# ModelCloud/GPTQModel

Hardware: NVIDIA H100
Metric: W4A16 g128 QuantLinear: decode tok/s + prefill TFLOPS vs HBM/TC roofline (higher is better)
Workload: dtype f16

## Files before the change

gptqmodel_b200/csrc/b2q_dequant.cuh:

```cuda
#pragma once
#include "b2q_common.cuh"

namespace b2q {

struct SZRaw {
  uint32_t s;
  uint32_t zw;
};

template <typename T, int BITS, bool ASYM>
__device__ __forceinline__ SZRaw load_sz(const T* __restrict__ scales, const uint32_t* __restrict__ qzeros, int g,
                                         int n, int N) {
  SZRaw r;
  r.s = *reinterpret_cast<const uint16_t*>(scales + (size_t)g * N + n);
  r.zw = 0;
  if (ASYM) {
    constexpr int PF = 32 / BITS;
    r.zw = qzeros[(size_t)g * (N / PF) + n / PF];
  }
  return r;
}

template <typename T, int BITS>
struct Dequant;

template <>
struct Dequant<__half, 4> {
  __device__ static __forceinline__ void run(const uint4& pv, uint32_t slo16, int zlo_i, uint32_t shi16, int zhi_i,
                                             uint4 (&lo)[2], uint4 (&hi)[2]) {
    const uint32_t slu = slo16 | (slo16 << 16), shu = shi16 | (shi16 << 16);
    const __half2 sl = *reinterpret_cast<const __half2*>(&slu), sh = *reinterpret_cast<const __half2*>(&shu);
    const __half2 zlo = __float2half2_rn(1024.f + (float)zlo_i);
    const __half2 zhi = __float2half2_rn(-(64.f + (float)zhi_i));
    const __half2 sixteenth = __float2half2_rn(0.0625f);
    const uint32_t w[4] = {pv.x, pv.y, pv.z, pv.w};
    uint32_t l[8], u[8];
#pragma unroll
    for (int s4 = 0; s4 < 4; ++s4) {
      uint32_t h[4];
      ET<__half>::unpack_w4(w[s4], h);
      __half2 v0 = __hmul2(__hsub2(*reinterpret_cast<__half2*>(&h[0]), zlo), sl);
      __half2 v1 = __hmul2(__hfma2(*reinterpret_cast<__half2*>(&h[1]), sixteenth, zhi), sh);
      __half2 v2 = __hmul2(__hsub2(*reinterpret_cast<__half2*>(&h[2]), zlo), sl);
      __half2 v3 = __hmul2(__hfma2(*reinterpret_cast<__half2*>(&h[3]), sixteenth, zhi), sh);
      l[2 * s4] = *reinterpret_cast<uint32_t*>(&v0);
      l[2 * s4 + 1] = *reinterpret_cast<uint32_t*>(&v2);
      u[2 * s4] = *reinterpret_cast<uint32_t*>(&v1);
      u[2 * s4 + 1] = *reinterpret_cast<uint32_t*>(&v3);
    }
    lo[0] = make_uint4(l[0], l[1], l[2], l[3]);
    lo[1] = make_uint4(l[4], l[5], l[6], l[7]);
    hi[0] = make_uint4(u[0], u[1], u[2], u[3]);
    hi[1] = make_uint4(u[4], u[5], u[6], u[7]);
  }
};

template <>
struct Dequant<__nv_bfloat16, 4> {
  __device__ static __forceinline__ void run(const uint4& pv, uint32_t slo16, int zlo_i, uint32_t shi16, int zhi_i,
                                             uint4 (&lo)[2], uint4 (&hi)[2]) {
    const uint32_t slu = slo16 | (slo16 << 16), shu = shi16 | (shi16 << 16);
    const __nv_bfloat162 sl = *reinterpret_cast<const __nv_bfloat162*>(&slu);
    const __nv_bfloat162 sh = *reinterpret_cast<const __nv_bfloat162*>(&shu);
    const __nv_bfloat162 zl = __float2bfloat162_rn(128.f + (float)zlo_i);
    const __nv_bfloat162 zh = __float2bfloat162_rn(128.f + (float)zhi_i);
    const uint32_t w[4] = {pv.x, pv.y, pv.z, pv.w};
    uint32_t l[8], u[8];
#pragma unroll
    for (int s4 = 0; s4 < 4; ++s4) {
      uint32_t h[4];
      ET<__nv_bfloat16>::unpack_w4(w[s4], h);
      __nv_bfloat162 v0 = __hmul2(__hsub2(*reinterpret_cast<__nv_bfloat162*>(&h[0]), zl), sl);
      __nv_bfloat162 v1 = __hmul2(__hsub2(*reinterpret_cast<__nv_bfloat162*>(&h[1]), zh), sh);
      __nv_bfloat162 v2 = __hmul2(__hsub2(*reinterpret_cast<__nv_bfloat162*>(&h[2]), zl), sl);
      __nv_bfloat162 v3 = __hmul2(__hsub2(*reinterpret_cast<__nv_bfloat162*>(&h[3]), zh), sh);
      l[2 * s4] = *reinterpret_cast<uint32_t*>(&v0);
      l[2 * s4 + 1] = *reinterpret_cast<uint32_t*>(&v2);
      u[2 * s4] = *reinterpret_cast<uint32_t*>(&v1);
      u[2 * s4 + 1] = *reinterpret_cast<uint32_t*>(&v3);
    }
    lo[0] = make_uint4(l[0], l[1], l[2], l[3]);
    lo[1] = make_uint4(l[4], l[5], l[6], l[7]);
    hi[0] = make_uint4(u[0], u[1], u[2], u[3]);
    hi[1] = make_uint4(u[4], u[5], u[6], u[7]);
  }
};

template <>
struct Dequant<__half, 8> {
  __device__ static __forceinline__ void run(const uint4& pv, uint32_t s16, int z, uint4 (&o)[2]) {
    const uint32_t s2u = s16 | (s16 << 16);
    const __half2 s2 = *reinterpret_cast<const __half2*>(&s2u);
    const __half2 zb = __float2half2_rn(1024.f + (float)z);
    const uint32_t w[4] = {pv.x, pv.y, pv.z, pv.w};
    uint32_t r[8];
#pragma unroll
    for (int t = 0; t < 4; ++t) {
      uint32_t p0 = __byte_perm(w[t], 0x64006400u, 0x7150);
      uint32_t p1 = __byte_perm(w[t], 0x64006400u, 0x7352);
      __half2 v0 = __hmul2(__hsub2(*reinterpret_cast<__half2*>(&p0), zb), s2);
      __half2 v1 = __hmul2(__hsub2(*reinterpret_cast<__half2*>(&p1), zb), s2);
      r[2 * t] = *reinterpret_cast<uint32_t*>(&v0);
      r[2 * t + 1] = *reinterpret_cast<uint32_t*>(&v1);
    }
    o[0] = make_uint4(r[0], r[1], r[2], r[3]);
    o[1] = make_uint4(r[4], r[5], r[6], r[7]);
  }
};

template <>
struct Dequant<__nv_bfloat16, 8> {
  __device__ static __forceinline__ void run(const uint4& pv, uint32_t s16, int z, uint4 (&o)[2]) {
    const float s = __uint_as_float(s16 << 16);
    const uint32_t w[4] = {pv.x, pv.y, pv.z, pv.w};
    uint32_t r[8];
#pragma unroll
    for (int t = 0; t < 4; ++t) {
      const float q0 = (float)((int)(w[t] & 0xFFu) - z), q1 = (float)((int)((w[t] >> 8) & 0xFFu) - z);
      const float q2 = (float)((int)((w[t] >> 16) & 0xFFu) - z), q3 = (float)((int)(w[t] >> 24) - z);
      r[2 * t] = ET<__nv_bfloat16>::pack2(q0 * s, q1 * s);
      r[2 * t + 1] = ET<__nv_bfloat16>::pack2(q2 * s, q3 * s);
    }
    o[0] = make_uint4(r[0], r[1], r[2], r[3]);
    o[1] = make_uint4(r[4], r[5], r[6], r[7]);
  }
};


}
```

gptqmodel_b200/csrc/b2q_gemm.cu:

```cuda
#include <cuda.h>

#include "b2q_common.cuh"
#include "b2q_dequant.cuh"
#include "b2q_gemm.cuh"
#include "b2q_internal.h"
#include "b2q_wgmma.cuh"

namespace b2q {

template <typename T, int BITS, bool ASYM, int STAGES>
__global__ void __launch_bounds__(G_THREADS, 1)
    gemm_kernel(const __grid_constant__ CUtensorMap tmap_x, const __grid_constant__ GemmSets S, int M, int K,
                int gshc) {
  using C = GemmCfg<BITS, STAGES>;
  using E = ET<T>;
  extern __shared__ uint8_t smem_raw[];
  const uint32_t smem_base = (smem_u32(smem_raw) + 1023u) & ~1023u;
  uint8_t* smem = smem_raw + (smem_base - smem_u32(smem_raw));

  const uint32_t sA = smem_base;
  const uint32_t sB = sA + STAGES * C::A_BYTES;
  const uint32_t sP = sB + STAGES * C::B_BYTES;
  const uint32_t sBar = sP + STAGES * C::P_BYTES;
  const uint32_t bar_full = sBar, bar_bready = sBar + 8 * STAGES, bar_empty = sBar + 16 * STAGES;

  int set = 0, tn = blockIdx.x;
  if (S.nsets > 1 && tn >= S.tn_end[0]) {
    set = (S.nsets > 2 && tn >= S.tn_end[1]) ? 2 : 1;
    tn -= S.tn_end[set - 1];
  }
  const int N = S.N[set];
  const uint4* __restrict__ packed = S.packed[set];
  const T* __restrict__ scales = reinterpret_cast<const T*>(S.scales[set]);
  const uint32_t* __restrict__ qzeros = S.qzeros[set];

  const int warp = threadIdx.x >> 5, lane = threadIdx.x & 31;
  const int NT = N >> 5;
  const int n0 = tn * G_BN, m0 = blockIdx.y * G_BM;
  const int nt0 = n0 >> 5;
  const int ntiles = min(4, NT - nt0);
  const int nkb = K / G_BK;

  if (threadIdx.x == 0) {
    prefetch_tmap(&tmap_x);
    for (int s = 0; s < STAGES; ++s) {
      mbar_init(bar_full + 8 * s, 1);
      mbar_init(bar_bready + 8 * s, G_DQ_THREADS);
      mbar_init(bar_empty + 8 * s, 1);
    }
    fence_mbar_init();
  }
  __syncthreads();

  if (warp == 8) {
    if (lane == 0) {
      const int FT = N >> 4, ft0 = n0 >> 4;
      const uint32_t pbytes4 = (uint32_t)min(8, FT - ft0) * 512u;
      const uint32_t pbytes8 = (uint32_t)ntiles * C::SUB * 512u;
      for (int kb = 0; kb < nkb; ++kb) {
        const int s = kb % STAGES;
        const uint32_t ph = (kb / STAGES) & 1;
        mbar_wait(bar_empty + 8 * s, ph ^ 1);
        const int g0 = (2 * kb) >> gshc, g1 = (2 * kb + 1) >> gshc;
        const int nrows = (g1 != g0) ? 2 : 1;
        const uint32_t sbytes = (uint32_t)min(G_BN, N - n0) * 2u, zbytes = ASYM ? sbytes / 4u : 0u;
        mbar_expect_tx(bar_full + 8 * s,
                       C::A_BYTES + (BITS == 4 ? pbytes4 + nrows * (sbytes + zbytes) : 2 * pbytes8));
        tma_load_2d(sA + s * C::A_BYTES, &tmap_x, bar_full + 8 * s, kb * G_BK, m0);
        if (BITS == 4) {
          bulk_load(sP + s * C::P_BYTES, packed + ((size_t)kb * FT + ft0) * 32, pbytes4, bar_full + 8 * s);
          for (int r = 0; r < nrows; ++r) {
            const int gr = r ? g1 : g0;
            bulk_load(sP + s * C::P_BYTES + 4096 + r * 320, scales + (size_t)gr * N + n0, sbytes, bar_full + 8 * s);
            if (ASYM)
              bulk_load(sP + s * C::P_BYTES + 4096 + r * 320 + 256, qzeros + (size_t)gr * (N >> 3) + (n0 >> 3),
                        zbytes, bar_full + 8 * s);
          }
        } else {
#pragma unroll
          for (int j = 0; j < 2; ++j)
            bulk_load(sP + s * C::P_BYTES + j * C::P_CHUNK_BYTES,
                      packed + ((size_t)(kb * 2 + j) * NT + nt0) * C::SUB * 32, pbytes8, bar_full + 8 * s);
        }
      }
    }
  } else if (warp < 4) {
    float acc[2][G_BN / 2];
#pragma unroll
    for (int mb = 0; mb < 2; ++mb)
#pragma unroll
      for (int i = 0; i < G_BN / 2; ++i) acc[mb][i] = 0.f;
    for (int kb = 0; kb < nkb; ++kb) {
      const int s = kb % STAGES;
      const uint32_t ph = (kb / STAGES) & 1;
      mbar_wait(bar_full + 8 * s, ph);
      mbar_wait(bar_bready + 8 * s, ph);
      wgmma_fence();
      const uint64_t bdesc = wgmma_desc_k_sw128(sB + s * C::B_BYTES);
      const uint64_t adesc = wgmma_desc_k_sw128(sA + s * C::A_BYTES);
#pragma unroll
      for (int k = 0; k < G_BK / 16; ++k) {
#pragma unroll
        for (int mb = 0; mb < 2; ++mb)
          Wgmma<E::FMT, G_BN>::mma(acc[mb], adesc + 512 * mb + 2 * k, bdesc + 2 * k, (kb | k) != 0 ? 1u : 0u);
      }
      wgmma_commit();
      wgmma_wait<1>();
      if (kb > 0 && threadIdx.x == 0) mbar_arrive(bar_empty + 8 * ((kb - 1) % STAGES));
    }
    wgmma_wait<0>();
#pragma unroll
    for (int mb = 0; mb < 2; ++mb) wgmma_fence_regs(acc[mb]);

    const T* __restrict__ bias = reinterpret_cast<const T*>(S.bias[set]);
    T* __restrict__ out = reinterpret_cast<T*>(S.out[set]);
#pragma unroll
    for (int mb = 0; mb < 2; ++mb) {
#pragma unroll
      for (int h = 0; h < 2; ++h) {
        const int row = m0 + 64 * mb + 16 * warp + (lane >> 2) + 8 * h;
        if (row >= M) continue;
        T* dst = out + (size_t)row * N;
#pragma unroll
        for (int j = 0; j < G_BN / 8; ++j) {
          const int col = n0 + 8 * j + 2 * (lane & 3);
          if (col >= N) continue;
          float f0 = acc[mb][4 * j + 2 * h], f1 = acc[mb][4 * j + 2 * h + 1];
          if (bias != nullptr) {
            f0 = E::to_f(E::from_f(f0)) + E::to_f(bias[col]);
            f1 = E::to_f(E::from_f(f1)) + E::to_f(bias[col + 1]);
          }
          *reinterpret_cast<uint32_t*>(dst + col) = E::pack2(f0, f1);
        }
      }
    }
  } else {
    const int t = threadIdx.x - G_MMA_THREADS;
    constexpr int PF = 32 / BITS;
    constexpr int ZSYM = 1 << (BITS - 1);
    if (BITS == 4) {
      const int lp = t & 31, g = lp >> 2, tt = lp & 3;
      int f[4];
      f[0] = (t >> 5) * 16 + g;
      f[1] = f[0] + 8;
      f[2] = f[0] + 64;
      f[3] = f[0] + 72;
      for (int kb = 0; kb < nkb; ++kb) {
        const int s = kb % STAGES;
        const uint32_t ph = (kb / STAGES) & 1;
        mbar_wait(bar_full + 8 * s, ph);
        const uint8_t* pst = smem + (sP - smem_base) + s * C::P_BYTES;
        const uint4* pj = reinterpret_cast<const uint4*>(pst);
        const int grow = ((2 * kb + (tt >> 1)) >> gshc) - ((2 * kb) >> gshc);
        const uint8_t* srow = pst + 4096 + grow * 320;
#pragma unroll
        for (int u = 0; u < 2; ++u) {
          const uint4 pv = pj[t + u * 128];
          const uint32_t s_lo = *reinterpret_cast<const uint16_t*>(srow + f[2 * u] * 2);
          const uint32_t s_hi = *reinterpret_cast<const uint16_t*>(srow + f[2 * u + 1] * 2);
          int zl = ZSYM, zh = ZSYM;
          if (ASYM) {
            const uint32_t zwl = *reinterpret_cast<const uint32_t*>(srow + 256 + (f[2 * u] >> 3) * 4);
            const uint32_t zwh = *reinterpret_cast<const uint32_t*>(srow + 256 + (f[2 * u + 1] >> 3) * 4);
            zl = (int)((zwl >> (4 * g)) & 15u);
            zh = (int)((zwh >> (4 * g)) & 15u);
          }
          uint4 lo[2], hi[2];
          Dequant<T, 4>::run(pv, s_lo, zl, s_hi, zh, lo, hi);
          const uint32_t sw = (uint32_t)g;
          const uint32_t rlo = sB + s * C::B_BYTES + f[2 * u] * 128;
          const uint32_t rhi = rlo + 8 * 128;
#pragma unroll
          for (int c = 0; c < 2; ++c) {
            const uint32_t off = (((uint32_t)(2 * tt + c)) ^ sw) << 4;
            asm volatile("st.shared.v4.u32 [%0], {%1,%2,%3,%4};" ::"r"(rlo + off), "r"(lo[c].x), "r"(lo[c].y),
                         "r"(lo[c].z), "r"(lo[c].w)
                         : "memory");
            asm volatile("st.shared.v4.u32 [%0], {%1,%2,%3,%4};" ::"r"(rhi + off), "r"(hi[c].x), "r"(hi[c].y),
                         "r"(hi[c].z), "r"(hi[c].w)
                         : "memory");
          }
        }
        fence_proxy_async_smem();
        mbar_arrive(bar_bready + 8 * s);
      }
    } else {
      const int n = n0 + t;
      const int nsafe = (n < N) ? n : 0;
      const int ntl = t >> 5;
      SZRaw cur[2], nxt[2];
      cur[0] = load_sz<T, BITS, ASYM>(scales, qzeros, 0, nsafe, N);
      cur[1] = load_sz<T, BITS, ASYM>(scales, qzeros, 1 >> gshc, nsafe, N);
      for (int kb = 0; kb < nkb; ++kb) {
        const int s = kb % STAGES;
        const uint32_t ph = (kb / STAGES) & 1;
        if (kb + 1 < nkb) {
          nxt[0] = load_sz<T, BITS, ASYM>(scales, qzeros, (2 * kb + 2) >> gshc, nsafe, N);
          nxt[1] = load_sz<T, BITS, ASYM>(scales, qzeros, (2 * kb + 3) >> gshc, nsafe, N);
        }
        mbar_wait(bar_full + 8 * s, ph);
        const uint32_t brow = sB + s * C::B_BYTES + t * 128;
        const uint32_t sw = (uint32_t)(t & 7);
#pragma unroll
        for (int j = 0; j < 2; ++j) {
          int z = ZSYM;
          if (ASYM) z = (int)((cur[j].zw >> (BITS * (nsafe % PF))) & ((1u << BITS) - 1));
          const uint4* pj = reinterpret_cast<const uint4*>(smem + (sP - smem_base) + s * C::P_BYTES +
                                                           j * C::P_CHUNK_BYTES);
#pragma unroll
          for (int h = 0; h < 2; ++h) {
            const uint4 pv = pj[(ntl * 2 + h) * 32 + lane];
            uint4 o[2];
            Dequant<T, 8>::run(pv, cur[j].s, z, o);
#pragma unroll
            for (int c = 0; c < 2; ++c) {
              const uint32_t addr = brow + (((uint32_t)(j * 4 + h * 2 + c) ^ sw) << 4);
              asm volatile("st.shared.v4.u32 [%0], {%1,%2,%3,%4};" ::"r"(addr), "r"(o[c].x), "r"(o[c].y),
                           "r"(o[c].z), "r"(o[c].w)
                           : "memory");
            }
          }
        }
        fence_proxy_async_smem();
        mbar_arrive(bar_bready + 8 * s);
        cur[0] = nxt[0];
        cur[1] = nxt[1];
      }
    }
  }
}

typedef CUresult (*EncodeTiledFn)(CUtensorMap*, CUtensorMapDataType, cuuint32_t, void*, const cuuint64_t*,
                                  const cuuint64_t*, const cuuint32_t*, const cuuint32_t*, CUtensorMapInterleave,
                                  CUtensorMapSwizzle, CUtensorMapL2promotion, CUtensorMapFloatOOBfill);

static EncodeTiledFn get_encode_fn() {
  static EncodeTiledFn fn = nullptr;
  if (fn == nullptr) {
    void* p = nullptr;
    cudaDriverEntryPointQueryResult qres;
    if (cudaGetDriverEntryPoint("cuTensorMapEncodeTiled", &p, cudaEnableDefault, &qres) == cudaSuccess &&
        qres == cudaDriverEntryPointSuccess)
      fn = reinterpret_cast<EncodeTiledFn>(p);
  }
  return fn;
}

int make_x_tmap_box(CUtensorMap* map, const void* x, int M, int K, int dtype, int box_rows) {
  struct Entry {
    const void* x;
    int M, K, dtype, box;
    CUtensorMap map;
  };
  constexpr int NCACHE = 16;
  static thread_local Entry cache[NCACHE];
  static thread_local int next = 0, filled = 0;
  for (int i = 0; i < filled; ++i) {
    const Entry& c = cache[i];
    if (c.x == x && c.M == M && c.K == K && c.dtype == dtype && c.box == box_rows) {
      *map = c.map;
      return 0;
    }
  }
  EncodeTiledFn enc = get_encode_fn();
  if (enc == nullptr) {
    set_error("b2q_gemm: cuTensorMapEncodeTiled not available from the driver");
    return -1;
  }
  cuuint64_t gdim[2] = {(cuuint64_t)K, (cuuint64_t)M};
  cuuint64_t gstride[1] = {(cuuint64_t)K * 2};
  cuuint32_t box[2] = {(cuuint32_t)G_BK, (cuuint32_t)box_rows};
  cuuint32_t estr[2] = {1, 1};
  CUresult r = enc(map, dtype == 0 ? CU_TENSOR_MAP_DATA_TYPE_FLOAT16 : CU_TENSOR_MAP_DATA_TYPE_BFLOAT16, 2,
                   const_cast<void*>(x), gdim, gstride, box, estr, CU_TENSOR_MAP_INTERLEAVE_NONE,
                   CU_TENSOR_MAP_SWIZZLE_128B, CU_TENSOR_MAP_L2_PROMOTION_L2_256B,
                   CU_TENSOR_MAP_FLOAT_OOB_FILL_NONE);
  if (r != CUDA_SUCCESS) {
    set_error("b2q_gemm: cuTensorMapEncodeTiled failed (%d) for x=%p M=%d K=%d box=%d", (int)r, x, M, K, box_rows);
    return -1;
  }
  Entry& e = cache[next];
  e.x = x;
  e.M = M;
  e.K = K;
  e.dtype = dtype;
  e.box = box_rows;
  e.map = *map;
  next = (next + 1) % NCACHE;
  if (filled < NCACHE) ++filled;
  return 0;
}

int make_x_tmap(CUtensorMap* map, const void* x, int M, int K, int dtype) {
  return make_x_tmap_box(map, x, M, K, dtype, 128);
}

int gemm_gshc(const MmArgs& a) {
  if (a.group_size == 32) return 0;
  if (a.group_size == 64) return 1;
  if (a.group_size == 128) return 2;
  return 31;
}


template <typename T, int BITS, bool ASYM, int STAGES>
static int launch_gemm_t(const MmArgs& a, const void* x, const GemmSets& S) {
  using C = GemmCfg<BITS, STAGES>;
  CUtensorMap tmap;
  if (make_x_tmap(&tmap, x, a.M, a.K, a.dtype) != 0) return -1;
  auto kern = gemm_kernel<T, BITS, ASYM, STAGES>;
  static int smem_opted[32] = {};
  if (int e = ensure_dyn_smem(kern, C::SMEM_BYTES, smem_opted, "b2q_gemm")) return e;
  dim3 grid(S.tn_end[S.nsets - 1], (a.M + G_BM - 1) / G_BM, 1);
  kern<<<grid, G_THREADS, C::SMEM_BYTES, a.stream>>>(tmap, S, a.M, a.K, gemm_gshc(a));
  return (int)cudaGetLastError();
}

static int launch_gemm_sets(const MmArgs& a, const void* x, const GemmSets& S) {
  const bool asym = S.qzeros[0] != nullptr;
#define B2Q_GEMM_CASE(T, BITS, ST) \
  (asym ? launch_gemm_t<T, BITS, true, ST>(a, x, S) : launch_gemm_t<T, BITS, false, ST>(a, x, S))
  if (a.dtype == 0) return a.bits == 4 ? B2Q_GEMM_CASE(__half, 4, 4) : B2Q_GEMM_CASE(__half, 8, 4);
  return a.bits == 4 ? B2Q_GEMM_CASE(__nv_bfloat16, 4, 4) : B2Q_GEMM_CASE(__nv_bfloat16, 8, 4);
#undef B2Q_GEMM_CASE
}

int launch_gemm_multi(const MmArgs& a, const void* x, int nsets, const void* const* packed, const void* const* scales,
                      const int32_t* const* qzeros, const void* const* bias, void* const* out, const int* Ns) {
  if (nsets < 1 || nsets > G_MAX_SETS) {
    set_error("b2q_gemm_multi: nsets=%d out of range (1..%d)", nsets, G_MAX_SETS);
    return -1;
  }
  if (a.K % G_BK != 0) {
    set_error("b2q_gemm_multi: K=%d must be a multiple of %d", a.K, G_BK);
    return -1;
  }
  GemmSets S = {};
  S.nsets = nsets;
  int tn = 0;
  for (int i = 0; i < nsets; ++i) {
    if (Ns[i] <= 0 || Ns[i] % 32 != 0 || packed[i] == nullptr || scales[i] == nullptr || out[i] == nullptr ||
        ((qzeros[i] != nullptr) != (qzeros[0] != nullptr))) {
      set_error("b2q_gemm_multi: set %d unsupported (N=%d; all sets share K, group size and symmetry)", i, Ns[i]);
      return -1;
    }
    tn += (Ns[i] + G_BN - 1) / G_BN;
    S.tn_end[i] = tn;
    S.N[i] = Ns[i];
    S.packed[i] = (const uint4*)packed[i];
    S.scales[i] = scales[i];
    S.qzeros[i] = (const uint32_t*)qzeros[i];
    S.bias[i] = bias[i];
    S.out[i] = out[i];
  }
  for (int i = nsets; i < G_MAX_SETS; ++i) S.tn_end[i] = tn;
  return launch_gemm_sets(a, x, S);
}

int launch_gemm(const MmArgs& a) {
  if (a.K % G_BK != 0) {
    set_error("b2q_gemm: K=%d must be a multiple of %d", a.K, G_BK);
    return -1;
  }
  const void* x = a.x;
  if (a.perm != nullptr) {
    const size_t need = (size_t)a.M * a.K * 2;
    if (a.workspace == nullptr || a.workspace_bytes < need) {
      set_error("b2q_gemm: act-order needs a %zu-byte workspace (got %zu)", need, a.workspace_bytes);
      return -1;
    }
    int e = launch_permute_cols(a.x, a.perm, a.workspace, a.M, a.K, a.stream);
    if (e != 0) return e;
    x = a.workspace;
  }
  if (a.M <= 128 && env().midm && midm_supported(a)) return launch_midm(a, x);
  const void* packed = a.packed;
  const void* scales = a.scales;
  const int32_t* qzeros = (const int32_t*)a.qzeros;
  const void* bias = a.bias;
  void* out = a.out;
  return launch_gemm_multi(a, x, 1, &packed, &scales, &qzeros, &bias, &out, &a.N);
}

}
```

gptqmodel_b200/csrc/b2q_gemm.cuh:

```cuda
#pragma once
#include "b2q_common.cuh"

namespace b2q {

constexpr int G_BM = 128;
constexpr int G_BN = 128;
constexpr int G_BK = 64;
constexpr int G_MMA_THREADS = 128;
constexpr int G_DQ_THREADS = 128;
constexpr int G_THREADS = G_MMA_THREADS + G_DQ_THREADS + 32;

template <int BITS, int STAGES>
struct GemmCfg {
  static constexpr int SUB = BITS / 4;
  static constexpr int A_BYTES = G_BM * G_BK * 2;
  static constexpr int B_BYTES = G_BN * G_BK * 2;
  static constexpr int P_CHUNK_BYTES = 4 * SUB * 512;
  static constexpr int P_BYTES = 2 * P_CHUNK_BYTES + (BITS == 4 ? 1024 : 0);
  static constexpr int STAGE_BYTES = A_BYTES + B_BYTES + P_BYTES;
  static constexpr int BAR_BYTES = 256;
  static constexpr int SMEM_BYTES = STAGES * STAGE_BYTES + BAR_BYTES + 1024;
  static_assert(SMEM_BYTES <= 227 * 1024, "dynamic shared memory of one CTA");
};

constexpr int G_MAX_SETS = 3;
struct GemmSets {
  int nsets;
  int tn_end[G_MAX_SETS];
  int N[G_MAX_SETS];
  const uint4* packed[G_MAX_SETS];
  const void* scales[G_MAX_SETS];
  const uint32_t* qzeros[G_MAX_SETS];
  const void* bias[G_MAX_SETS];
  void* out[G_MAX_SETS];
};

}
```

gptqmodel_b200/csrc/b2q_wgmma.cuh:

```cuda
#pragma once
#include "b2q_common.cuh"

namespace b2q {

__device__ __forceinline__ uint64_t wgmma_desc_k_sw128(uint32_t saddr) {
  return (uint64_t)((saddr & 0x3FFFFu) >> 4) | (1ull << 16) | (64ull << 32) | (1ull << 62);
}
__device__ __forceinline__ void wgmma_fence() { asm volatile("wgmma.fence.sync.aligned;" ::: "memory"); }
__device__ __forceinline__ void wgmma_commit() { asm volatile("wgmma.commit_group.sync.aligned;" ::: "memory"); }
template <int N>
__device__ __forceinline__ void wgmma_wait() {
  asm volatile("wgmma.wait_group.sync.aligned %0;" ::"n"(N) : "memory");
}
template <int R>
__device__ __forceinline__ void wgmma_fence_regs(float (&d)[R]) {
#pragma unroll
  for (int i = 0; i < R; ++i) asm volatile("" : "+f"(d[i])::"memory");
}

template <int FMT, int N>
struct Wgmma;
template <>
struct Wgmma<0, 16> {
  __device__ static __forceinline__ void mma(float (&d)[8], uint64_t a, uint64_t b, uint32_t accumulate) {
    asm volatile(
        "{ .reg .pred p; setp.ne.b32 p, %10, 0;\n"
        "  wgmma.mma_async.sync.aligned.m64n16k16.f32.f16.f16 {%0,%1,%2,%3,%4,%5,%6,%7}, %8, %9, p, 1, 1, 0, 0; }"
        : "+f"(d[0]), "+f"(d[1]), "+f"(d[2]), "+f"(d[3]), "+f"(d[4]), "+f"(d[5]), "+f"(d[6]), "+f"(d[7])
        : "l"(a), "l"(b), "r"(accumulate));
  }
};
template <>
struct Wgmma<0, 32> {
  __device__ static __forceinline__ void mma(float (&d)[16], uint64_t a, uint64_t b, uint32_t accumulate) {
    asm volatile(
        "{ .reg .pred p; setp.ne.b32 p, %18, 0;\n"
        "  wgmma.mma_async.sync.aligned.m64n32k16.f32.f16.f16 {%0,%1,%2,%3,%4,%5,%6,%7,%8,%9,%10,%11,%12,%13,%14,%15}, %16, %17, p, 1, 1, 0, 0; }"
        : "+f"(d[0]), "+f"(d[1]), "+f"(d[2]), "+f"(d[3]), "+f"(d[4]), "+f"(d[5]), "+f"(d[6]), "+f"(d[7]), "+f"(d[8]), "+f"(d[9]), "+f"(d[10]), "+f"(d[11]), "+f"(d[12]), "+f"(d[13]), "+f"(d[14]), "+f"(d[15])
        : "l"(a), "l"(b), "r"(accumulate));
  }
};
template <>
struct Wgmma<0, 64> {
  __device__ static __forceinline__ void mma(float (&d)[32], uint64_t a, uint64_t b, uint32_t accumulate) {
    asm volatile(
        "{ .reg .pred p; setp.ne.b32 p, %34, 0;\n"
        "  wgmma.mma_async.sync.aligned.m64n64k16.f32.f16.f16 {%0,%1,%2,%3,%4,%5,%6,%7,%8,%9,%10,%11,%12,%13,%14,%15,%16,%17,%18,%19,%20,%21,%22,%23,%24,%25,%26,%27,%28,%29,%30,%31}, %32, %33, p, 1, 1, 0, 0; }"
        : "+f"(d[0]), "+f"(d[1]), "+f"(d[2]), "+f"(d[3]), "+f"(d[4]), "+f"(d[5]), "+f"(d[6]), "+f"(d[7]), "+f"(d[8]), "+f"(d[9]), "+f"(d[10]), "+f"(d[11]), "+f"(d[12]), "+f"(d[13]), "+f"(d[14]), "+f"(d[15]), "+f"(d[16]), "+f"(d[17]), "+f"(d[18]), "+f"(d[19]), "+f"(d[20]), "+f"(d[21]), "+f"(d[22]), "+f"(d[23]), "+f"(d[24]), "+f"(d[25]), "+f"(d[26]), "+f"(d[27]), "+f"(d[28]), "+f"(d[29]), "+f"(d[30]), "+f"(d[31])
        : "l"(a), "l"(b), "r"(accumulate));
  }
};
template <>
struct Wgmma<0, 128> {
  __device__ static __forceinline__ void mma(float (&d)[64], uint64_t a, uint64_t b, uint32_t accumulate) {
    asm volatile(
        "{ .reg .pred p; setp.ne.b32 p, %66, 0;\n"
        "  wgmma.mma_async.sync.aligned.m64n128k16.f32.f16.f16 {%0,%1,%2,%3,%4,%5,%6,%7,%8,%9,%10,%11,%12,%13,%14,%15,%16,%17,%18,%19,%20,%21,%22,%23,%24,%25,%26,%27,%28,%29,%30,%31,%32,%33,%34,%35,%36,%37,%38,%39,%40,%41,%42,%43,%44,%45,%46,%47,%48,%49,%50,%51,%52,%53,%54,%55,%56,%57,%58,%59,%60,%61,%62,%63}, %64, %65, p, 1, 1, 0, 0; }"
        : "+f"(d[0]), "+f"(d[1]), "+f"(d[2]), "+f"(d[3]), "+f"(d[4]), "+f"(d[5]), "+f"(d[6]), "+f"(d[7]), "+f"(d[8]), "+f"(d[9]), "+f"(d[10]), "+f"(d[11]), "+f"(d[12]), "+f"(d[13]), "+f"(d[14]), "+f"(d[15]), "+f"(d[16]), "+f"(d[17]), "+f"(d[18]), "+f"(d[19]), "+f"(d[20]), "+f"(d[21]), "+f"(d[22]), "+f"(d[23]), "+f"(d[24]), "+f"(d[25]), "+f"(d[26]), "+f"(d[27]), "+f"(d[28]), "+f"(d[29]), "+f"(d[30]), "+f"(d[31]), "+f"(d[32]), "+f"(d[33]), "+f"(d[34]), "+f"(d[35]), "+f"(d[36]), "+f"(d[37]), "+f"(d[38]), "+f"(d[39]), "+f"(d[40]), "+f"(d[41]), "+f"(d[42]), "+f"(d[43]), "+f"(d[44]), "+f"(d[45]), "+f"(d[46]), "+f"(d[47]), "+f"(d[48]), "+f"(d[49]), "+f"(d[50]), "+f"(d[51]), "+f"(d[52]), "+f"(d[53]), "+f"(d[54]), "+f"(d[55]), "+f"(d[56]), "+f"(d[57]), "+f"(d[58]), "+f"(d[59]), "+f"(d[60]), "+f"(d[61]), "+f"(d[62]), "+f"(d[63])
        : "l"(a), "l"(b), "r"(accumulate));
  }
};
template <>
struct Wgmma<1, 16> {
  __device__ static __forceinline__ void mma(float (&d)[8], uint64_t a, uint64_t b, uint32_t accumulate) {
    asm volatile(
        "{ .reg .pred p; setp.ne.b32 p, %10, 0;\n"
        "  wgmma.mma_async.sync.aligned.m64n16k16.f32.bf16.bf16 {%0,%1,%2,%3,%4,%5,%6,%7}, %8, %9, p, 1, 1, 0, 0; }"
        : "+f"(d[0]), "+f"(d[1]), "+f"(d[2]), "+f"(d[3]), "+f"(d[4]), "+f"(d[5]), "+f"(d[6]), "+f"(d[7])
        : "l"(a), "l"(b), "r"(accumulate));
  }
};
template <>
struct Wgmma<1, 32> {
  __device__ static __forceinline__ void mma(float (&d)[16], uint64_t a, uint64_t b, uint32_t accumulate) {
    asm volatile(
        "{ .reg .pred p; setp.ne.b32 p, %18, 0;\n"
        "  wgmma.mma_async.sync.aligned.m64n32k16.f32.bf16.bf16 {%0,%1,%2,%3,%4,%5,%6,%7,%8,%9,%10,%11,%12,%13,%14,%15}, %16, %17, p, 1, 1, 0, 0; }"
        : "+f"(d[0]), "+f"(d[1]), "+f"(d[2]), "+f"(d[3]), "+f"(d[4]), "+f"(d[5]), "+f"(d[6]), "+f"(d[7]), "+f"(d[8]), "+f"(d[9]), "+f"(d[10]), "+f"(d[11]), "+f"(d[12]), "+f"(d[13]), "+f"(d[14]), "+f"(d[15])
        : "l"(a), "l"(b), "r"(accumulate));
  }
};
template <>
struct Wgmma<1, 64> {
  __device__ static __forceinline__ void mma(float (&d)[32], uint64_t a, uint64_t b, uint32_t accumulate) {
    asm volatile(
        "{ .reg .pred p; setp.ne.b32 p, %34, 0;\n"
        "  wgmma.mma_async.sync.aligned.m64n64k16.f32.bf16.bf16 {%0,%1,%2,%3,%4,%5,%6,%7,%8,%9,%10,%11,%12,%13,%14,%15,%16,%17,%18,%19,%20,%21,%22,%23,%24,%25,%26,%27,%28,%29,%30,%31}, %32, %33, p, 1, 1, 0, 0; }"
        : "+f"(d[0]), "+f"(d[1]), "+f"(d[2]), "+f"(d[3]), "+f"(d[4]), "+f"(d[5]), "+f"(d[6]), "+f"(d[7]), "+f"(d[8]), "+f"(d[9]), "+f"(d[10]), "+f"(d[11]), "+f"(d[12]), "+f"(d[13]), "+f"(d[14]), "+f"(d[15]), "+f"(d[16]), "+f"(d[17]), "+f"(d[18]), "+f"(d[19]), "+f"(d[20]), "+f"(d[21]), "+f"(d[22]), "+f"(d[23]), "+f"(d[24]), "+f"(d[25]), "+f"(d[26]), "+f"(d[27]), "+f"(d[28]), "+f"(d[29]), "+f"(d[30]), "+f"(d[31])
        : "l"(a), "l"(b), "r"(accumulate));
  }
};
template <>
struct Wgmma<1, 128> {
  __device__ static __forceinline__ void mma(float (&d)[64], uint64_t a, uint64_t b, uint32_t accumulate) {
    asm volatile(
        "{ .reg .pred p; setp.ne.b32 p, %66, 0;\n"
        "  wgmma.mma_async.sync.aligned.m64n128k16.f32.bf16.bf16 {%0,%1,%2,%3,%4,%5,%6,%7,%8,%9,%10,%11,%12,%13,%14,%15,%16,%17,%18,%19,%20,%21,%22,%23,%24,%25,%26,%27,%28,%29,%30,%31,%32,%33,%34,%35,%36,%37,%38,%39,%40,%41,%42,%43,%44,%45,%46,%47,%48,%49,%50,%51,%52,%53,%54,%55,%56,%57,%58,%59,%60,%61,%62,%63}, %64, %65, p, 1, 1, 0, 0; }"
        : "+f"(d[0]), "+f"(d[1]), "+f"(d[2]), "+f"(d[3]), "+f"(d[4]), "+f"(d[5]), "+f"(d[6]), "+f"(d[7]), "+f"(d[8]), "+f"(d[9]), "+f"(d[10]), "+f"(d[11]), "+f"(d[12]), "+f"(d[13]), "+f"(d[14]), "+f"(d[15]), "+f"(d[16]), "+f"(d[17]), "+f"(d[18]), "+f"(d[19]), "+f"(d[20]), "+f"(d[21]), "+f"(d[22]), "+f"(d[23]), "+f"(d[24]), "+f"(d[25]), "+f"(d[26]), "+f"(d[27]), "+f"(d[28]), "+f"(d[29]), "+f"(d[30]), "+f"(d[31]), "+f"(d[32]), "+f"(d[33]), "+f"(d[34]), "+f"(d[35]), "+f"(d[36]), "+f"(d[37]), "+f"(d[38]), "+f"(d[39]), "+f"(d[40]), "+f"(d[41]), "+f"(d[42]), "+f"(d[43]), "+f"(d[44]), "+f"(d[45]), "+f"(d[46]), "+f"(d[47]), "+f"(d[48]), "+f"(d[49]), "+f"(d[50]), "+f"(d[51]), "+f"(d[52]), "+f"(d[53]), "+f"(d[54]), "+f"(d[55]), "+f"(d[56]), "+f"(d[57]), "+f"(d[58]), "+f"(d[59]), "+f"(d[60]), "+f"(d[61]), "+f"(d[62]), "+f"(d[63])
        : "l"(a), "l"(b), "r"(accumulate));
  }
};

}
```

Before: 612.3.

## Dequantize weights into registers and feed wgmma from registers, dropping the dequant smem stage

Replaces the producer/dequant/MMA warp split with two consumer warpgroups. Each one dequantizes packed weights straight into register fragments, using shuffles to arrange them, and issues register-operand wgmma, so the dequantized B tile is no longer stored in shared memory and the bready barrier goes away. This apparently computes the transposed product, with weights as the A operand. Other changes: the pipeline deepens from 4 to 8 stages, the output is staged through the activation ring for 16-byte stores, and a rows_fast grid ordering is chosen when weight bytes dominate. The costs are more register pressure and shuffle work, and a new 16-byte output alignment requirement.

After: 612.8 (median of 6 runs). No clear change (+0.1%).

```diff
diff --git a/gptqmodel_b200/csrc/b2q_dequant.cuh b/gptqmodel_b200/csrc/b2q_dequant.cuh
--- a/gptqmodel_b200/csrc/b2q_dequant.cuh
+++ b/gptqmodel_b200/csrc/b2q_dequant.cuh
@@ -21,32 +21,109 @@
   return r;
 }
 
+template <typename T>
+struct DqW4;
+template <>
+struct DqW4<__half> {
+  __half2 sl, sh, zlo, zhi;
+  __device__ __forceinline__ DqW4(uint32_t slo16, int zlo_i, uint32_t shi16, int zhi_i) {
+    const uint32_t slu = slo16 | (slo16 << 16), shu = shi16 | (shi16 << 16);
+    sl = *reinterpret_cast<const __half2*>(&slu);
+    sh = *reinterpret_cast<const __half2*>(&shu);
+    zlo = __float2half2_rn(1024.f + (float)zlo_i);
+    zhi = __float2half2_rn(-(64.f + (float)zhi_i));
+  }
+  __device__ __forceinline__ void word(uint32_t w, uint32_t (&v)[4]) const {
+    const __half2 sixteenth = __float2half2_rn(0.0625f);
+    uint32_t h[4];
+    ET<__half>::unpack_w4(w, h);
+    __half2 v0 = __hmul2(__hsub2(*reinterpret_cast<__half2*>(&h[0]), zlo), sl);
+    __half2 v1 = __hmul2(__hfma2(*reinterpret_cast<__half2*>(&h[1]), sixteenth, zhi), sh);
+    __half2 v2 = __hmul2(__hsub2(*reinterpret_cast<__half2*>(&h[2]), zlo), sl);
+    __half2 v3 = __hmul2(__hfma2(*reinterpret_cast<__half2*>(&h[3]), sixteenth, zhi), sh);
+    v[0] = *reinterpret_cast<uint32_t*>(&v0);
+    v[1] = *reinterpret_cast<uint32_t*>(&v1);
+    v[2] = *reinterpret_cast<uint32_t*>(&v2);
+    v[3] = *reinterpret_cast<uint32_t*>(&v3);
+  }
+};
+template <>
+struct DqW4<__nv_bfloat16> {
+  __nv_bfloat162 sl, sh, zl, zh;
+  __device__ __forceinline__ DqW4(uint32_t slo16, int zlo_i, uint32_t shi16, int zhi_i) {
+    const uint32_t slu = slo16 | (slo16 << 16), shu = shi16 | (shi16 << 16);
+    sl = *reinterpret_cast<const __nv_bfloat162*>(&slu);
+    sh = *reinterpret_cast<const __nv_bfloat162*>(&shu);
+    zl = __float2bfloat162_rn(128.f + (float)zlo_i);
+    zh = __float2bfloat162_rn(128.f + (float)zhi_i);
+  }
+  __device__ __forceinline__ void word(uint32_t w, uint32_t (&v)[4]) const {
+    uint32_t h[4];
+    ET<__nv_bfloat16>::unpack_w4(w, h);
+    __nv_bfloat162 v0 = __hmul2(__hsub2(*reinterpret_cast<__nv_bfloat162*>(&h[0]), zl), sl);
+    __nv_bfloat162 v1 = __hmul2(__hsub2(*reinterpret_cast<__nv_bfloat162*>(&h[1]), zh), sh);
+    __nv_bfloat162 v2 = __hmul2(__hsub2(*reinterpret_cast<__nv_bfloat162*>(&h[2]), zl), sl);
+    __nv_bfloat162 v3 = __hmul2(__hsub2(*reinterpret_cast<__nv_bfloat162*>(&h[3]), zh), sh);
+    v[0] = *reinterpret_cast<uint32_t*>(&v0);
+    v[1] = *reinterpret_cast<uint32_t*>(&v1);
+    v[2] = *reinterpret_cast<uint32_t*>(&v2);
+    v[3] = *reinterpret_cast<uint32_t*>(&v3);
+  }
+};
+
+template <typename T>
+struct DqW8;
+template <>
+struct DqW8<__half> {
+  __half2 s2, zb;
+  __device__ __forceinline__ DqW8(uint32_t s16, int z) {
+    const uint32_t s2u = s16 | (s16 << 16);
+    s2 = *reinterpret_cast<const __half2*>(&s2u);
+    zb = __float2half2_rn(1024.f + (float)z);
+  }
+  __device__ __forceinline__ void word(uint32_t w, uint32_t (&r)[2]) const {
+    uint32_t p0 = __byte_perm(w, 0x64006400u, 0x7150);
+    uint32_t p1 = __byte_perm(w, 0x64006400u, 0x7352);
+    __half2 v0 = __hmul2(__hsub2(*reinterpret_cast<__half2*>(&p0), zb), s2);
+    __half2 v1 = __hmul2(__hsub2(*reinterpret_cast<__half2*>(&p1), zb), s2);
+    r[0] = *reinterpret_cast<uint32_t*>(&v0);
+    r[1] = *reinterpret_cast<uint32_t*>(&v1);
+  }
+};
+template <>
+struct DqW8<__nv_bfloat16> {
+  float s;
+  int z;
+  __device__ __forceinline__ DqW8(uint32_t s16, int z_) {
+    s = __uint_as_float(s16 << 16);
+    z = z_;
+  }
+  __device__ __forceinline__ void word(uint32_t w, uint32_t (&r)[2]) const {
+    const float q0 = (float)((int)(w & 0xFFu) - z), q1 = (float)((int)((w >> 8) & 0xFFu) - z);
+    const float q2 = (float)((int)((w >> 16) & 0xFFu) - z), q3 = (float)((int)(w >> 24) - z);
+    r[0] = ET<__nv_bfloat16>::pack2(q0 * s, q1 * s);
+    r[1] = ET<__nv_bfloat16>::pack2(q2 * s, q3 * s);
+  }
+};
+
 template <typename T, int BITS>
 struct Dequant;
 
-template <>
-struct Dequant<__half, 4> {
+template <typename T>
+struct Dequant<T, 4> {
   __device__ static __forceinline__ void run(const uint4& pv, uint32_t slo16, int zlo_i, uint32_t shi16, int zhi_i,
                                              uint4 (&lo)[2], uint4 (&hi)[2]) {
-    const uint32_t slu = slo16 | (slo16 << 16), shu = shi16 | (shi16 << 16);
-    const __half2 sl = *reinterpret_cast<const __half2*>(&slu), sh = *reinterpret_cast<const __half2*>(&shu);
-    const __half2 zlo = __float2half2_rn(1024.f + (float)zlo_i);
-    const __half2 zhi = __float2half2_rn(-(64.f + (float)zhi_i));
-    const __half2 sixteenth = __float2half2_rn(0.0625f);
+    const DqW4<T> d(slo16, zlo_i, shi16, zhi_i);
     const uint32_t w[4] = {pv.x, pv.y, pv.z, pv.w};
     uint32_t l[8], u[8];
 #pragma unroll
     for (int s4 = 0; s4 < 4; ++s4) {
-      uint32_t h[4];
-      ET<__half>::unpack_w4(w[s4], h);
-      __half2 v0 = __hmul2(__hsub2(*reinterpret_cast<__half2*>(&h[0]), zlo), sl);
-      __half2 v1 = __hmul2(__hfma2(*reinterpret_cast<__half2*>(&h[1]), sixteenth, zhi), sh);
-      __half2 v2 = __hmul2(__hsub2(*reinterpret_cast<__half2*>(&h[2]), zlo), sl);
-      __half2 v3 = __hmul2(__hfma2(*reinterpret_cast<__half2*>(&h[3]), sixteenth, zhi), sh);
-      l[2 * s4] = *reinterpret_cast<uint32_t*>(&v0);
-      l[2 * s4 + 1] = *reinterpret_cast<uint32_t*>(&v2);
-      u[2 * s4] = *reinterpret_cast<uint32_t*>(&v1);
-      u[2 * s4 + 1] = *reinterpret_cast<uint32_t*>(&v3);
+      uint32_t v[4];
+      d.word(w[s4], v);
+      l[2 * s4] = v[0];
+      l[2 * s4 + 1] = v[2];
+      u[2 * s4] = v[1];
+      u[2 * s4 + 1] = v[3];
     }
     lo[0] = make_uint4(l[0], l[1], l[2], l[3]);
     lo[1] = make_uint4(l[4], l[5], l[6], l[7]);
@@ -55,71 +132,18 @@
   }
 };
 
-template <>
-struct Dequant<__nv_bfloat16, 4> {
-  __device__ static __forceinline__ void run(const uint4& pv, uint32_t slo16, int zlo_i, uint32_t shi16, int zhi_i,
-                                             uint4 (&lo)[2], uint4 (&hi)[2]) {
-    const uint32_t slu = slo16 | (slo16 << 16), shu = shi16 | (shi16 << 16);
-    const __nv_bfloat162 sl = *reinterpret_cast<const __nv_bfloat162*>(&slu);
-    const __nv_bfloat162 sh = *reinterpret_cast<const __nv_bfloat162*>(&shu);
-    const __nv_bfloat162 zl = __float2bfloat162_rn(128.f + (float)zlo_i);
-    const __nv_bfloat162 zh = __float2bfloat162_rn(128.f + (float)zhi_i);
-    const uint32_t w[4] = {pv.x, pv.y, pv.z, pv.w};
-    uint32_t l[8], u[8];
-#pragma unroll
-    for (int s4 = 0; s4 < 4; ++s4) {
-      uint32_t h[4];
-      ET<__nv_bfloat16>::unpack_w4(w[s4], h);
-      __nv_bfloat162 v0 = __hmul2(__hsub2(*reinterpret_cast<__nv_bfloat162*>(&h[0]), zl), sl);
-      __nv_bfloat162 v1 = __hmul2(__hsub2(*reinterpret_cast<__nv_bfloat162*>(&h[1]), zh), sh);
-      __nv_bfloat162 v2 = __hmul2(__hsub2(*reinterpret_cast<__nv_bfloat162*>(&h[2]), zl), sl);
-      __nv_bfloat162 v3 = __hmul2(__hsub2(*reinterpret_cast<__nv_bfloat162*>(&h[3]), zh), sh);
-      l[2 * s4] = *reinterpret_cast<uint32_t*>(&v0);
-      l[2 * s4 + 1] = *reinterpret_cast<uint32_t*>(&v2);
-      u[2 * s4] = *reinterpret_cast<uint32_t*>(&v1);
-      u[2 * s4 + 1] = *reinterpret_cast<uint32_t*>(&v3);
-    }
-    lo[0] = make_uint4(l[0], l[1], l[2], l[3]);
-    lo[1] = make_uint4(l[4], l[5], l[6], l[7]);
-    hi[0] = make_uint4(u[0], u[1], u[2], u[3]);
-    hi[1] = make_uint4(u[4], u[5], u[6], u[7]);
-  }
-};
-
-template <>
-struct Dequant<__half, 8> {
+template <typename T>
+struct Dequant<T, 8> {
   __device__ static __forceinline__ void run(const uint4& pv, uint32_t s16, int z, uint4 (&o)[2]) {
-    const uint32_t s2u = s16 | (s16 << 16);
-    const __half2 s2 = *reinterpret_cast<const __half2*>(&s2u);
-    const __half2 zb = __float2half2_rn(1024.f + (float)z);
+    const DqW8<T> d(s16, z);
     const uint32_t w[4] = {pv.x, pv.y, pv.z, pv.w};
     uint32_t r[8];
 #pragma unroll
     for (int t = 0; t < 4; ++t) {
-      uint32_t p0 = __byte_perm(w[t], 0x64006400u, 0x7150);
-      uint32_t p1 = __byte_perm(w[t], 0x64006400u, 0x7352);
-      __half2 v0 = __hmul2(__hsub2(*reinterpret_cast<__half2*>(&p0), zb), s2);
-      __half2 v1 = __hmul2(__hsub2(*reinterpret_cast<__half2*>(&p1), zb), s2);
-      r[2 * t] = *reinterpret_cast<uint32_t*>(&v0);
-      r[2 * t + 1] = *reinterpret_cast<uint32_t*>(&v1);
-    }
-    o[0] = make_uint4(r[0], r[1], r[2], r[3]);
-    o[1] = make_uint4(r[4], r[5], r[6], r[7]);
-  }
-};
-
-template <>
-struct Dequant<__nv_bfloat16, 8> {
-  __device__ static __forceinline__ void run(const uint4& pv, uint32_t s16, int z, uint4 (&o)[2]) {
-    const float s = __uint_as_float(s16 << 16);
-    const uint32_t w[4] = {pv.x, pv.y, pv.z, pv.w};
-    uint32_t r[8];
-#pragma unroll
-    for (int t = 0; t < 4; ++t) {
-      const float q0 = (float)((int)(w[t] & 0xFFu) - z), q1 = (float)((int)((w[t] >> 8) & 0xFFu) - z);
-      const float q2 = (float)((int)((w[t] >> 16) & 0xFFu) - z), q3 = (float)((int)(w[t] >> 24) - z);
-      r[2 * t] = ET<__nv_bfloat16>::pack2(q0 * s, q1 * s);
-      r[2 * t + 1] = ET<__nv_bfloat16>::pack2(q2 * s, q3 * s);
+      uint32_t v[2];
+      d.word(w[t], v);
+      r[2 * t] = v[0];
+      r[2 * t + 1] = v[1];
     }
     o[0] = make_uint4(r[0], r[1], r[2], r[3]);
     o[1] = make_uint4(r[4], r[5], r[6], r[7]);
diff --git a/gptqmodel_b200/csrc/b2q_gemm.cu b/gptqmodel_b200/csrc/b2q_gemm.cu
--- a/gptqmodel_b200/csrc/b2q_gemm.cu
+++ b/gptqmodel_b200/csrc/b2q_gemm.cu
@@ -8,23 +8,49 @@
 
 namespace b2q {
 
+__device__ __forceinline__ uint4 lds128(uint32_t addr) {
+  uint4 v;
+  asm volatile("ld.shared.v4.u32 {%0,%1,%2,%3}, [%4];" : "=r"(v.x), "=r"(v.y), "=r"(v.z), "=r"(v.w) : "r"(addr) : "memory");
+  return v;
+}
+
+template <uint32_t SEL0, uint32_t SEL1, bool OWN_IS_T>
+__device__ __forceinline__ void a_words(const uint4& v, int own, int t, int src0, int stride, uint32_t (&cw)[4]) {
+  const bool ohi = (own & 2) != 0, oodd = (own & 1) != 0;
+  const uint32_t wa = ohi ? v.y : v.x, wa2 = ohi ? v.x : v.y;
+  const uint32_t wb = ohi ? v.w : v.z, wb2 = ohi ? v.z : v.w;
+  const uint32_t sa = oodd ? SEL1 : SEL0, sb = oodd ? SEL0 : SEL1;
+  uint32_t rv[4];
+#pragma unroll
+  for (int r = 0; r < 4; ++r) {
+    const uint32_t x = __byte_perm((r & 2) ? wa2 : wa, (r & 2) ? wb2 : wb, (r & 1) ? sb : sa);
+    rv[r] = (OWN_IS_T && r == 0) ? x : __shfl_sync(0xffffffffu, x, src0 + stride * (t ^ r));
+  }
+  const bool t1 = (t & 1) != 0, t2 = (t & 2) != 0;
+  const uint32_t p0 = t1 ? rv[1] : rv[0], p1 = t1 ? rv[0] : rv[1];
+  const uint32_t p2 = t1 ? rv[3] : rv[2], p3 = t1 ? rv[2] : rv[3];
+  cw[0] = t2 ? p2 : p0;
+  cw[1] = t2 ? p3 : p1;
+  cw[2] = t2 ? p0 : p2;
+  cw[3] = t2 ? p1 : p3;
+}
+
 template <typename T, int BITS, bool ASYM, int STAGES>
 __global__ void __launch_bounds__(G_THREADS, 1)
     gemm_kernel(const __grid_constant__ CUtensorMap tmap_x, const __grid_constant__ GemmSets S, int M, int K,
-                int gshc) {
+                int gshc, int rows_fast) {
   using C = GemmCfg<BITS, STAGES>;
   using E = ET<T>;
   extern __shared__ uint8_t smem_raw[];
   const uint32_t smem_base = (smem_u32(smem_raw) + 1023u) & ~1023u;
   uint8_t* smem = smem_raw + (smem_base - smem_u32(smem_raw));
 
-  const uint32_t sA = smem_base;
-  const uint32_t sB = sA + STAGES * C::A_BYTES;
-  const uint32_t sP = sB + STAGES * C::B_BYTES;
+  const uint32_t sX = smem_base;
+  const uint32_t sP = sX + STAGES * C::X_BYTES;
   const uint32_t sBar = sP + STAGES * C::P_BYTES;
-  const uint32_t bar_full = sBar, bar_bready = sBar + 8 * STAGES, bar_empty = sBar + 16 * STAGES;
-
-  int set = 0, tn = blockIdx.x;
+  const uint32_t bar_full = sBar, bar_empty = sBar + 8 * STAGES;
+
+  int set = 0, tn = rows_fast ? blockIdx.y : blockIdx.x;
   if (S.nsets > 1 && tn >= S.tn_end[0]) {
     set = (S.nsets > 2 && tn >= S.tn_end[1]) ? 2 : 1;
     tn -= S.tn_end[set - 1];
@@ -36,7 +62,7 @@
 
   const int warp = threadIdx.x >> 5, lane = threadIdx.x & 31;
   const int NT = N >> 5;
-  const int n0 = tn * G_BN, m0 = blockIdx.y * G_BM;
+  const int n0 = tn * G_BN, m0 = (rows_fast ? blockIdx.x : blockIdx.y) * G_BM;
   const int nt0 = n0 >> 5;
   const int ntiles = min(4, NT - nt0);
   const int nkb = K / G_BK;
@@ -45,8 +71,7 @@
     prefetch_tmap(&tmap_x);
     for (int s = 0; s < STAGES; ++s) {
       mbar_init(bar_full + 8 * s, 1);
-      mbar_init(bar_bready + 8 * s, G_DQ_THREADS);
-      mbar_init(bar_empty + 8 * s, 1);
+      mbar_init(bar_empty + 8 * s, G_CONSUMERS);
     }
     fence_mbar_init();
   }
@@ -65,8 +90,8 @@
         const int nrows = (g1 != g0) ? 2 : 1;
         const uint32_t sbytes = (uint32_t)min(G_BN, N - n0) * 2u, zbytes = ASYM ? sbytes / 4u : 0u;
         mbar_expect_tx(bar_full + 8 * s,
-                       C::A_BYTES + (BITS == 4 ? pbytes4 + nrows * (sbytes + zbytes) : 2 * pbytes8));
-        tma_load_2d(sA + s * C::A_BYTES, &tmap_x, bar_full + 8 * s, kb * G_BK, m0);
+                       C::X_BYTES + (BITS == 4 ? pbytes4 + nrows * (sbytes + zbytes) : 2 * pbytes8));
+        tma_load_2d(sX + s * C::X_BYTES, &tmap_x, bar_full + 8 * s, kb * G_BK, m0);
         if (BITS == 4) {
           bulk_load(sP + s * C::P_BYTES, packed + ((size_t)kb * FT + ft0) * 32, pbytes4, bar_full + 8 * s);
           for (int r = 0; r < nrows; ++r) {
@@ -84,149 +109,140 @@
         }
       }
     }
-  } else if (warp < 4) {
-    float acc[2][G_BN / 2];
-#pragma unroll
-    for (int mb = 0; mb < 2; ++mb)
-#pragma unroll
-      for (int i = 0; i < G_BN / 2; ++i) acc[mb][i] = 0.f;
-    for (int kb = 0; kb < nkb; ++kb) {
-      const int s = kb % STAGES;
-      const uint32_t ph = (kb / STAGES) & 1;
-      mbar_wait(bar_full + 8 * s, ph);
-      mbar_wait(bar_bready + 8 * s, ph);
-      wgmma_fence();
-      const uint64_t bdesc = wgmma_desc_k_sw128(sB + s * C::B_BYTES);
-      const uint64_t adesc = wgmma_desc_k_sw128(sA + s * C::A_BYTES);
-#pragma unroll
-      for (int k = 0; k < G_BK / 16; ++k) {
-#pragma unroll
-        for (int mb = 0; mb < 2; ++mb)
-          Wgmma<E::FMT, G_BN>::mma(acc[mb], adesc + 512 * mb + 2 * k, bdesc + 2 * k, (kb | k) != 0 ? 1u : 0u);
+    return;
+  }
+
+  const int g = lane >> 2, t = lane & 3;
+  const int fw = 64 * (warp >> 2) + 16 * (warp & 3);
+  const int fa = n0 + fw < N ? fw : 0;
+  const int f_lo = fa + g;
+  constexpr int ZSYM = 1 << (BITS - 1);
+  SZRaw sz_even[2][2], sz_odd[2][2];
+
+  auto load_sz8 = [&](int kb, SZRaw (&o)[2][2]) {
+#pragma unroll
+    for (int r = 0; r < 2; ++r)
+#pragma unroll
+      for (int h = 0; h < 2; ++h)
+        o[r][h] = load_sz<T, BITS, ASYM>(scales, qzeros, (2 * kb + h) >> gshc, n0 + f_lo + 8 * r, N);
+  };
+  if (BITS == 8) load_sz8(0, sz_even);
+
+  float acc[G_BM / 2];
+#pragma unroll
+  for (int i = 0; i < G_BM / 2; ++i) acc[i] = 0.f;
+  uint32_t a_even[4][4], a_odd[4][4];
+
+  auto step = [&](int kb, uint32_t (&af)[4][4], const SZRaw (&cur)[2][2], SZRaw (&nxt)[2][2]) {
+    const int s = kb % STAGES;
+    const uint32_t ph = (kb / STAGES) & 1;
+    if (BITS == 8) load_sz8(min(kb + 1, nkb - 1), nxt);
+    mbar_wait(bar_full + 8 * s, ph);
+    const uint32_t sPs = sP + s * C::P_BYTES;
+    const uint8_t* pst = smem + (sPs - smem_base);
+    if (BITS == 4) {
+      uint32_t cw[4];
+      a_words<0x6240u, 0x7351u, true>(lds128(sPs + ((fa >> 4) * 32 + lane) * 16), t, t, 4 * g, 1, cw);
+      const int grow1 = ((2 * kb + 1) >> gshc) - ((2 * kb) >> gshc);
+#pragma unroll
+      for (int h = 0; h < 2; ++h) {
+        const uint8_t* srow = pst + 4096 + (h ? grow1 : 0) * 320;
+        const uint32_t s_lo = *reinterpret_cast<const uint16_t*>(srow + f_lo * 2);
+        const uint32_t s_hi = *reinterpret_cast<const uint16_t*>(srow + (f_lo + 8) * 2);
+        int zl = ZSYM, zh = ZSYM;
+        if (ASYM) {
+          zl = (int)((*reinterpret_cast<const uint32_t*>(srow + 256 + (f_lo >> 3) * 4) >> (4 * g)) & 15u);
+          zh = (int)((*reinterpret_cast<const uint32_t*>(srow + 256 + ((f_lo + 8) >> 3) * 4) >> (4 * g)) & 15u);
+        }
+        const DqW4<T> d(s_lo, zl, s_hi, zh);
+        d.word(cw[2 * h], af[2 * h]);
+        d.word(cw[2 * h + 1], af[2 * h + 1]);
       }
-      wgmma_commit();
-      wgmma_wait<1>();
-      if (kb > 0 && threadIdx.x == 0) mbar_arrive(bar_empty + 8 * ((kb - 1) % STAGES));
-    }
-    wgmma_wait<0>();
-#pragma unroll
-    for (int mb = 0; mb < 2; ++mb) wgmma_fence_regs(acc[mb]);
-
-    const T* __restrict__ bias = reinterpret_cast<const T*>(S.bias[set]);
-    T* __restrict__ out = reinterpret_cast<T*>(S.out[set]);
-#pragma unroll
-    for (int mb = 0; mb < 2; ++mb) {
+    } else {
+      const int ls = lane >> 3, lr = (fa & 31) + (lane & 7);
+      const uint32_t pj = sPs + (ls >> 1) * C::P_CHUNK_BYTES + (((fa >> 5) * 2 + (ls & 1)) * 32 + lr) * 16;
+      uint32_t clo[4], chi[4];
+      a_words<0x5410u, 0x7632u, false>(lds128(pj), ls, t, g, 8, clo);
+      a_words<0x5410u, 0x7632u, false>(lds128(pj + 8 * 16), ls, t, g, 8, chi);
 #pragma unroll
       for (int h = 0; h < 2; ++h) {
-        const int row = m0 + 64 * mb + 16 * warp + (lane >> 2) + 8 * h;
-        if (row >= M) continue;
-        T* dst = out + (size_t)row * N;
-#pragma unroll
-        for (int j = 0; j < G_BN / 8; ++j) {
-          const int col = n0 + 8 * j + 2 * (lane & 3);
-          if (col >= N) continue;
-          float f0 = acc[mb][4 * j + 2 * h], f1 = acc[mb][4 * j + 2 * h + 1];
-          if (bias != nullptr) {
-            f0 = E::to_f(E::from_f(f0)) + E::to_f(bias[col]);
-            f1 = E::to_f(E::from_f(f1)) + E::to_f(bias[col + 1]);
-          }
-          *reinterpret_cast<uint32_t*>(dst + col) = E::pack2(f0, f1);
+        int zl = ZSYM, zh = ZSYM;
+        if (ASYM) {
+          zl = (int)((cur[0][h].zw >> (8 * (g & 3))) & 255u);
+          zh = (int)((cur[1][h].zw >> (8 * (g & 3))) & 255u);
+        }
+        const DqW8<T> dl(cur[0][h].s, zl), dh(cur[1][h].s, zh);
+#pragma unroll
+        for (int jj = 0; jj < 2; ++jj) {
+          uint32_t* a = af[2 * h + jj];
+          uint32_t r[2];
+          dl.word(clo[2 * h + jj], r);
+          a[0] = r[0];
+          a[2] = r[1];
+          dh.word(chi[2 * h + jj], r);
+          a[1] = r[0];
+          a[3] = r[1];
         }
       }
     }
-  } else {
-    const int t = threadIdx.x - G_MMA_THREADS;
-    constexpr int PF = 32 / BITS;
-    constexpr int ZSYM = 1 << (BITS - 1);
-    if (BITS == 4) {
-      const int lp = t & 31, g = lp >> 2, tt = lp & 3;
-      int f[4];
-      f[0] = (t >> 5) * 16 + g;
-      f[1] = f[0] + 8;
-      f[2] = f[0] + 64;
-      f[3] = f[0] + 72;
-      for (int kb = 0; kb < nkb; ++kb) {
-        const int s = kb % STAGES;
-        const uint32_t ph = (kb / STAGES) & 1;
-        mbar_wait(bar_full + 8 * s, ph);
-        const uint8_t* pst = smem + (sP - smem_base) + s * C::P_BYTES;
-        const uint4* pj = reinterpret_cast<const uint4*>(pst);
-        const int grow = ((2 * kb + (tt >> 1)) >> gshc) - ((2 * kb) >> gshc);
-        const uint8_t* srow = pst + 4096 + grow * 320;
-#pragma unroll
-        for (int u = 0; u < 2; ++u) {
-          const uint4 pv = pj[t + u * 128];
-          const uint32_t s_lo = *reinterpret_cast<const uint16_t*>(srow + f[2 * u] * 2);
-          const uint32_t s_hi = *reinterpret_cast<const uint16_t*>(srow + f[2 * u + 1] * 2);
-          int zl = ZSYM, zh = ZSYM;
-          if (ASYM) {
-            const uint32_t zwl = *reinterpret_cast<const uint32_t*>(srow + 256 + (f[2 * u] >> 3) * 4);
-            const uint32_t zwh = *reinterpret_cast<const uint32_t*>(srow + 256 + (f[2 * u + 1] >> 3) * 4);
-            zl = (int)((zwl >> (4 * g)) & 15u);
-            zh = (int)((zwh >> (4 * g)) & 15u);
-          }
-          uint4 lo[2], hi[2];
-          Dequant<T, 4>::run(pv, s_lo, zl, s_hi, zh, lo, hi);
-          const uint32_t sw = (uint32_t)g;
-          const uint32_t rlo = sB + s * C::B_BYTES + f[2 * u] * 128;
-          const uint32_t rhi = rlo + 8 * 128;
-#pragma unroll
-          for (int c = 0; c < 2; ++c) {
-            const uint32_t off = (((uint32_t)(2 * tt + c)) ^ sw) << 4;
-            asm volatile("st.shared.v4.u32 [%0], {%1,%2,%3,%4};" ::"r"(rlo + off), "r"(lo[c].x), "r"(lo[c].y),
-                         "r"(lo[c].z), "r"(lo[c].w)
-                         : "memory");
-            asm volatile("st.shared.v4.u32 [%0], {%1,%2,%3,%4};" ::"r"(rhi + off), "r"(hi[c].x), "r"(hi[c].y),
-                         "r"(hi[c].z), "r"(hi[c].w)
-                         : "memory");
-          }
-        }
-        fence_proxy_async_smem();
-        mbar_arrive(bar_bready + 8 * s);
+#pragma unroll
+    for (int j = 0; j < 4; ++j) wgmma_fence_regs(af[j]);
+    wgmma_fence_regs(acc);
+    wgmma_fence();
+    const uint64_t xdesc = wgmma_desc_k_sw128(sX + s * C::X_BYTES);
+#pragma unroll
+    for (int j = 0; j < G_BK / 16; ++j)
+      WgmmaRS<E::FMT, G_BM>::mma(acc, af[j], xdesc + 2 * j, (kb | j) != 0 ? 1u : 0u);
+    wgmma_commit();
+    wgmma_wait<1>();
+    if (kb > 0 && (threadIdx.x & 127) == 0) mbar_arrive(bar_empty + 8 * ((kb - 1) % STAGES));
+  };
+  int kb = 0;
+  for (; kb + 1 < nkb; kb += 2) {
+    step(kb, a_even, sz_even, sz_odd);
+    step(kb + 1, a_odd, sz_odd, sz_even);
+  }
+  if (kb < nkb) step(kb, a_even, sz_even, sz_odd);
+  wgmma_wait<0>();
+  wgmma_fence_regs(acc);
+
+  constexpr int NCONS = G_CONSUMERS * 128;
+  asm volatile("bar.sync 1, %0;" ::"n"(NCONS) : "memory");
+  const uint32_t sO = smem_base;
+  {
+    const int i = lane >> 3, r = lane & 7;
+    const uint32_t row_addr = sO + (uint32_t)((8 * (i >> 1) + r) * C::OUT_PITCH + (fw + 8 * (i & 1)) * 2);
+#pragma unroll
+    for (int jp = 0; jp < G_BM / 16; ++jp) {
+      const float* d0 = acc + 8 * jp;
+      asm volatile("stmatrix.sync.aligned.m8n8.x4.trans.shared.b16 [%0], {%1, %2, %3, %4};" ::"r"(
+                       row_addr + (uint32_t)(jp * 16 * C::OUT_PITCH)),
+                   "r"(E::pack2(d0[0], d0[1])), "r"(E::pack2(d0[2], d0[3])), "r"(E::pack2(d0[4], d0[5])),
+                   "r"(E::pack2(d0[6], d0[7]))
+                   : "memory");
+    }
+  }
+  asm volatile("bar.sync 1, %0;" ::"n"(NCONS) : "memory");
+  const T* __restrict__ bias = reinterpret_cast<const T*>(S.bias[set]);
+  T* __restrict__ out = reinterpret_cast<T*>(S.out[set]);
+  for (int q = threadIdx.x; q < G_BM * (G_BN / 8); q += NCONS) {
+    const int row = q >> 4, col = n0 + 8 * (q & 15);
+    if (m0 + row >= M || col >= N) continue;
+    uint4 v;
+    asm volatile("ld.shared.v4.u32 {%0,%1,%2,%3}, [%4];"
+                 : "=r"(v.x), "=r"(v.y), "=r"(v.z), "=r"(v.w)
+                 : "r"(sO + (uint32_t)(row * C::OUT_PITCH + (q & 15) * 16))
+                 : "memory");
+    if (bias != nullptr) {
+      uint32_t w[4] = {v.x, v.y, v.z, v.w};
+#pragma unroll
+      for (int e = 0; e < 4; ++e) {
+        const T* h = reinterpret_cast<const T*>(&w[e]);
+        w[e] = E::pack2(E::to_f(h[0]) + E::to_f(bias[col + 2 * e]), E::to_f(h[1]) + E::to_f(bias[col + 2 * e + 1]));
       }
-    } else {
-      const int n = n0 + t;
-      const int nsafe = (n < N) ? n : 0;
-      const int ntl = t >> 5;
-      SZRaw cur[2], nxt[2];
-      cur[0] = load_sz<T, BITS, ASYM>(scales, qzeros, 0, nsafe, N);
-      cur[1] = load_sz<T, BITS, ASYM>(scales, qzeros, 1 >> gshc, nsafe, N);
-      for (int kb = 0; kb < nkb; ++kb) {
-        const int s = kb % STAGES;
-        const uint32_t ph = (kb / STAGES) & 1;
-        if (kb + 1 < nkb) {
-          nxt[0] = load_sz<T, BITS, ASYM>(scales, qzeros, (2 * kb + 2) >> gshc, nsafe, N);
-          nxt[1] = load_sz<T, BITS, ASYM>(scales, qzeros, (2 * kb + 3) >> gshc, nsafe, N);
-        }
-        mbar_wait(bar_full + 8 * s, ph);
-        const uint32_t brow = sB + s * C::B_BYTES + t * 128;
-        const uint32_t sw = (uint32_t)(t & 7);
-#pragma unroll
-        for (int j = 0; j < 2; ++j) {
-          int z = ZSYM;
-          if (ASYM) z = (int)((cur[j].zw >> (BITS * (nsafe % PF))) & ((1u << BITS) - 1));
-          const uint4* pj = reinterpret_cast<const uint4*>(smem + (sP - smem_base) + s * C::P_BYTES +
-                                                           j * C::P_CHUNK_BYTES);
-#pragma unroll
-          for (int h = 0; h < 2; ++h) {
-            const uint4 pv = pj[(ntl * 2 + h) * 32 + lane];
-            uint4 o[2];
-            Dequant<T, 8>::run(pv, cur[j].s, z, o);
-#pragma unroll
-            for (int c = 0; c < 2; ++c) {
-              const uint32_t addr = brow + (((uint32_t)(j * 4 + h * 2 + c) ^ sw) << 4);
-              asm volatile("st.shared.v4.u32 [%0], {%1,%2,%3,%4};" ::"r"(addr), "r"(o[c].x), "r"(o[c].y),
-                           "r"(o[c].z), "r"(o[c].w)
-                           : "memory");
-            }
-          }
-        }
-        fence_proxy_async_smem();
-        mbar_arrive(bar_bready + 8 * s);
-        cur[0] = nxt[0];
-        cur[1] = nxt[1];
-      }
-    }
+      v = make_uint4(w[0], w[1], w[2], w[3]);
+    }
+    *reinterpret_cast<uint4*>(out + (size_t)(m0 + row) * N + col) = v;
   }
 }
 
@@ -311,8 +327,12 @@
   auto kern = gemm_kernel<T, BITS, ASYM, STAGES>;
   static int smem_opted[32] = {};
   if (int e = ensure_dyn_smem(kern, C::SMEM_BYTES, smem_opted, "b2q_gemm")) return e;
-  dim3 grid(S.tn_end[S.nsets - 1], (a.M + G_BM - 1) / G_BM, 1);
-  kern<<<grid, G_THREADS, C::SMEM_BYTES, a.stream>>>(tmap, S, a.M, a.K, gemm_gshc(a));
+  const int mblocks = (a.M + G_BM - 1) / G_BM, ncols = S.tn_end[S.nsets - 1];
+  int ntotal = 0;
+  for (int i = 0; i < S.nsets; ++i) ntotal += S.N[i];
+  const int rows_fast = (size_t)ntotal * BITS / 8 > (size_t)a.M * 2 && ncols <= 65535;
+  const dim3 grid(rows_fast ? mblocks : ncols, rows_fast ? ncols : mblocks, 1);
+  kern<<<grid, G_THREADS, C::SMEM_BYTES, a.stream>>>(tmap, S, a.M, a.K, gemm_gshc(a), rows_fast);
   return (int)cudaGetLastError();
 }
 
@@ -320,8 +340,8 @@
   const bool asym = S.qzeros[0] != nullptr;
 #define B2Q_GEMM_CASE(T, BITS, ST) \
   (asym ? launch_gemm_t<T, BITS, true, ST>(a, x, S) : launch_gemm_t<T, BITS, false, ST>(a, x, S))
-  if (a.dtype == 0) return a.bits == 4 ? B2Q_GEMM_CASE(__half, 4, 4) : B2Q_GEMM_CASE(__half, 8, 4);
-  return a.bits == 4 ? B2Q_GEMM_CASE(__nv_bfloat16, 4, 4) : B2Q_GEMM_CASE(__nv_bfloat16, 8, 4);
+  if (a.dtype == 0) return a.bits == 4 ? B2Q_GEMM_CASE(__half, 4, 8) : B2Q_GEMM_CASE(__half, 8, 8);
+  return a.bits == 4 ? B2Q_GEMM_CASE(__nv_bfloat16, 4, 8) : B2Q_GEMM_CASE(__nv_bfloat16, 8, 8);
 #undef B2Q_GEMM_CASE
 }
 
@@ -340,8 +360,9 @@
   int tn = 0;
   for (int i = 0; i < nsets; ++i) {
     if (Ns[i] <= 0 || Ns[i] % 32 != 0 || packed[i] == nullptr || scales[i] == nullptr || out[i] == nullptr ||
-        ((qzeros[i] != nullptr) != (qzeros[0] != nullptr))) {
-      set_error("b2q_gemm_multi: set %d unsupported (N=%d; all sets share K, group size and symmetry)", i, Ns[i]);
+        (reinterpret_cast<uintptr_t>(out[i]) & 15) || ((qzeros[i] != nullptr) != (qzeros[0] != nullptr))) {
+      set_error("b2q_gemm_multi: set %d unsupported (N=%d, 16-byte aligned out; all sets share K, group size and "
+                "symmetry)", i, Ns[i]);
       return -1;
     }
     tn += (Ns[i] + G_BN - 1) / G_BN;
diff --git a/gptqmodel_b200/csrc/b2q_gemm.cuh b/gptqmodel_b200/csrc/b2q_gemm.cuh
--- a/gptqmodel_b200/csrc/b2q_gemm.cuh
+++ b/gptqmodel_b200/csrc/b2q_gemm.cuh
@@ -6,20 +6,21 @@
 constexpr int G_BM = 128;
 constexpr int G_BN = 128;
 constexpr int G_BK = 64;
-constexpr int G_MMA_THREADS = 128;
-constexpr int G_DQ_THREADS = 128;
-constexpr int G_THREADS = G_MMA_THREADS + G_DQ_THREADS + 32;
+constexpr int G_CONSUMERS = 2;
+constexpr int G_THREADS = G_CONSUMERS * 128 + 32;
 
 template <int BITS, int STAGES>
 struct GemmCfg {
   static constexpr int SUB = BITS / 4;
-  static constexpr int A_BYTES = G_BM * G_BK * 2;
-  static constexpr int B_BYTES = G_BN * G_BK * 2;
+  static constexpr int X_BYTES = G_BM * G_BK * 2;
   static constexpr int P_CHUNK_BYTES = 4 * SUB * 512;
   static constexpr int P_BYTES = 2 * P_CHUNK_BYTES + (BITS == 4 ? 1024 : 0);
-  static constexpr int STAGE_BYTES = A_BYTES + B_BYTES + P_BYTES;
+  static constexpr int STAGE_BYTES = X_BYTES + P_BYTES;
   static constexpr int BAR_BYTES = 256;
   static constexpr int SMEM_BYTES = STAGES * STAGE_BYTES + BAR_BYTES + 1024;
+  static constexpr int OUT_PITCH = G_BN * 2 + 16;
+  static_assert(G_BM * OUT_PITCH <= STAGES * X_BYTES, "the output tile reuses the activation ring");
+  static_assert(2 * STAGES * 8 <= BAR_BYTES, "mbarrier area");
   static_assert(SMEM_BYTES <= 227 * 1024, "dynamic shared memory of one CTA");
 };
 
diff --git a/gptqmodel_b200/csrc/b2q_wgmma.cuh b/gptqmodel_b200/csrc/b2q_wgmma.cuh
--- a/gptqmodel_b200/csrc/b2q_wgmma.cuh
+++ b/gptqmodel_b200/csrc/b2q_wgmma.cuh
@@ -16,6 +16,11 @@
 __device__ __forceinline__ void wgmma_fence_regs(float (&d)[R]) {
 #pragma unroll
   for (int i = 0; i < R; ++i) asm volatile("" : "+f"(d[i])::"memory");
+}
+template <int R>
+__device__ __forceinline__ void wgmma_fence_regs(uint32_t (&a)[R]) {
+#pragma unroll
+  for (int i = 0; i < R; ++i) asm volatile("" : "+r"(a[i])::"memory");
 }
 
 template <int FMT, int N>
@@ -101,4 +106,27 @@
   }
 };
 
+template <int FMT, int N>
+struct WgmmaRS;
+template <>
+struct WgmmaRS<0, 128> {
+  __device__ static __forceinline__ void mma(float (&d)[64], const uint32_t (&a)[4], uint64_t b, uint32_t accumulate) {
+    asm volatile(
+        "{ .reg .pred p; setp.ne.b32 p, %69, 0;\n"
+        "  wgmma.mma_async.sync.aligned.m64n128k16.f32.f16.f16 {%0,%1,%2,%3,%4,%5,%6,%7,%8,%9,%10,%11,%12,%13,%14,%15,%16,%17,%18,%19,%20,%21,%22,%23,%24,%25,%26,%27,%28,%29,%30,%31,%32,%33,%34,%35,%36,%37,%38,%39,%40,%41,%42,%43,%44,%45,%46,%47,%48,%49,%50,%51,%52,%53,%54,%55,%56,%57,%58,%59,%60,%61,%62,%63}, {%64,%65,%66,%67}, %68, p, 1, 1, 0; }"
+        : "+f"(d[0]), "+f"(d[1]), "+f"(d[2]), "+f"(d[3]), "+f"(d[4]), "+f"(d[5]), "+f"(d[6]), "+f"(d[7]), "+f"(d[8]), "+f"(d[9]), "+f"(d[10]), "+f"(d[11]), "+f"(d[12]), "+f"(d[13]), "+f"(d[14]), "+f"(d[15]), "+f"(d[16]), "+f"(d[17]), "+f"(d[18]), "+f"(d[19]), "+f"(d[20]), "+f"(d[21]), "+f"(d[22]), "+f"(d[23]), "+f"(d[24]), "+f"(d[25]), "+f"(d[26]), "+f"(d[27]), "+f"(d[28]), "+f"(d[29]), "+f"(d[30]), "+f"(d[31]), "+f"(d[32]), "+f"(d[33]), "+f"(d[34]), "+f"(d[35]), "+f"(d[36]), "+f"(d[37]), "+f"(d[38]), "+f"(d[39]), "+f"(d[40]), "+f"(d[41]), "+f"(d[42]), "+f"(d[43]), "+f"(d[44]), "+f"(d[45]), "+f"(d[46]), "+f"(d[47]), "+f"(d[48]), "+f"(d[49]), "+f"(d[50]), "+f"(d[51]), "+f"(d[52]), "+f"(d[53]), "+f"(d[54]), "+f"(d[55]), "+f"(d[56]), "+f"(d[57]), "+f"(d[58]), "+f"(d[59]), "+f"(d[60]), "+f"(d[61]), "+f"(d[62]), "+f"(d[63])
+        : "r"(a[0]), "r"(a[1]), "r"(a[2]), "r"(a[3]), "l"(b), "r"(accumulate));
+  }
+};
+template <>
+struct WgmmaRS<1, 128> {
+  __device__ static __forceinline__ void mma(float (&d)[64], const uint32_t (&a)[4], uint64_t b, uint32_t accumulate) {
+    asm volatile(
+        "{ .reg .pred p; setp.ne.b32 p, %69, 0;\n"
+        "  wgmma.mma_async.sync.aligned.m64n128k16.f32.bf16.bf16 {%0,%1,%2,%3,%4,%5,%6,%7,%8,%9,%10,%11,%12,%13,%14,%15,%16,%17,%18,%19,%20,%21,%22,%23,%24,%25,%26,%27,%28,%29,%30,%31,%32,%33,%34,%35,%36,%37,%38,%39,%40,%41,%42,%43,%44,%45,%46,%47,%48,%49,%50,%51,%52,%53,%54,%55,%56,%57,%58,%59,%60,%61,%62,%63}, {%64,%65,%66,%67}, %68, p, 1, 1, 0; }"
+        : "+f"(d[0]), "+f"(d[1]), "+f"(d[2]), "+f"(d[3]), "+f"(d[4]), "+f"(d[5]), "+f"(d[6]), "+f"(d[7]), "+f"(d[8]), "+f"(d[9]), "+f"(d[10]), "+f"(d[11]), "+f"(d[12]), "+f"(d[13]), "+f"(d[14]), "+f"(d[15]), "+f"(d[16]), "+f"(d[17]), "+f"(d[18]), "+f"(d[19]), "+f"(d[20]), "+f"(d[21]), "+f"(d[22]), "+f"(d[23]), "+f"(d[24]), "+f"(d[25]), "+f"(d[26]), "+f"(d[27]), "+f"(d[28]), "+f"(d[29]), "+f"(d[30]), "+f"(d[31]), "+f"(d[32]), "+f"(d[33]), "+f"(d[34]), "+f"(d[35]), "+f"(d[36]), "+f"(d[37]), "+f"(d[38]), "+f"(d[39]), "+f"(d[40]), "+f"(d[41]), "+f"(d[42]), "+f"(d[43]), "+f"(d[44]), "+f"(d[45]), "+f"(d[46]), "+f"(d[47]), "+f"(d[48]), "+f"(d[49]), "+f"(d[50]), "+f"(d[51]), "+f"(d[52]), "+f"(d[53]), "+f"(d[54]), "+f"(d[55]), "+f"(d[56]), "+f"(d[57]), "+f"(d[58]), "+f"(d[59]), "+f"(d[60]), "+f"(d[61]), "+f"(d[62]), "+f"(d[63])
+        : "r"(a[0]), "r"(a[1]), "r"(a[2]), "r"(a[3]), "l"(b), "r"(accumulate));
+  }
+};
+
 }
```
